# CompVis/stable-diffusion

Hardware: AMD Instinct MI355X
Metric: 512x512 images/sec, SD-v1-4 50-step PLMS CFG=7.5 (higher is better)
Workload: dtype f16

## Files before the change

### stable-diffusion_amd/csrc/conv3halo.hip

```cpp
#include "igemm_dev.h"

namespace sdmi {
namespace {

template <int BM, int BN, int WARPS_M, int WARPS_N, int NS>
__global__ void __launch_bounds__(WARPS_M* WARPS_N * 64) conv3halo_kernel(const IGemmParams p, const int tiles_m,
                                                                           const int tiles_n, const int chunks_per_split) {
#if defined(__HIP_DEVICE_COMPILE__)
  constexpr int NT = WARPS_M * WARPS_N * 64;
  constexpr int RPP = NT / 8;
  constexpr int PB = BN / RPP;
  constexpr int WTM = BM / WARPS_M, WTN = BN / WARPS_N;
  constexpr int TM = WTM / 32, TN = WTN / 32;
  constexpr int HPMAX = (BM / 64 + 2) * 66;
  constexpr int AHP = (HPMAX + RPP - 1) / RPP;
  constexpr int HALO_BYTES = AHP * RPP * 128;
  constexpr int BSTAGE = BN * 128;
  constexpr int LDS_BYTES = 2 * HALO_BYTES + NS * BSTAGE;
  constexpr int LASTA = 10 - NS;
  constexpr int PA = (AHP + LASTA) / (LASTA + 1);
  constexpr int KS = BK / 16;
  constexpr int G = (TM * TN >= 4) ? 1 : 2;
  constexpr int U = KS / G;
  constexpr int MPU = G * TM * TN;
  static_assert(PB >= 1 && TM >= 1 && TN >= 1 && RPP % 16 == 0 && NS >= 2 && NS <= 9, "tile/wave shape");
  static_assert(LDS_BYTES <= 160 * 1024, "LDS budget");

  __shared__ __attribute__((aligned(16))) unsigned char smem[LDS_BYTES];

  const int nblk = gridDim.x;
  const int bid = blockIdx.x;
  const int q8 = nblk >> 3, r8 = nblk & 7, xcd = bid & 7;
  const int wgid = (xcd < r8 ? xcd * (q8 + 1) : r8 * (q8 + 1) + (xcd - r8) * q8) + (bid >> 3);
  const int tiles_mn = tiles_m * tiles_n;
  const int split = wgid / tiles_mn;
  const int tmn = wgid - split * tiles_mn;
  int tile_m, tile_n;
  if (p.tile_n_fastest) { tile_m = tmn / tiles_n; tile_n = tmn - tile_m * tiles_n; }
  else { tile_n = tmn / tiles_m; tile_m = tmn - tile_n * tiles_m; }
  const int m0 = tile_m * BM, n0 = tile_n * BN;
  const int nch = (p.c0 + p.c1 + p.c2) / BK;
  const int c_begin = split * chunks_per_split;
  const int c_end = min(nch, c_begin + chunks_per_split);
  if (c_begin >= c_end) return;

  const int tid = threadIdx.x;
  SDMI_STAMP(dbg_t0);
  const int lane = tid & 63;
  const int wave = tid >> 6;
  const int cpos = tid & 7, lrow = tid >> 3;
  const int gch = cpos ^ ((lrow >> 1) & 7);
  const int wave_u = __builtin_amdgcn_readfirstlane(wave);
  const int wm = wave / WARPS_N, wn = wave - wm * WARPS_N;
  const int l31 = lane & 31, lg = lane >> 5;
  const int rsw = (l31 >> 1) & 7;

  const int W = p.Wout, H = p.Hout, HW = H * W, W2 = W + 2, ld = p.lda0;
  const int bimg = m0 / HW;
  const int THI = p.halo_thi;
  const int HPI = (THI + 2) * W2;
  const int y0 = p.halo_ipt > 1 ? 0 : (m0 - bimg * HW) >> p.log2w;
  const int HP = p.halo_ipt * HPI;
  constexpr int OOB = (int)0x80000000;

  int hvoff[AHP];
#pragma unroll
  for (int q = 0; q < AHP; ++q) {
    const int hp = q * RPP + lrow;
    const int ip = fast_div(hp, p.magic_hpi), hr = hp - ip * HPI;
    const int hy = fast_div(hr, p.magic_w2), hx = hr - hy * W2;
    const int y = y0 + hy - 1, x = hx - 1;
    const bool valid = hp < HP && y >= 0 && y < H && x >= 0 && x < W;
    hvoff[q] = valid ? ((((bimg + ip) * H + y) * W + x) * ld + gch * 8) * 2 : OOB;
  }
  int b_off[PB];
#pragma unroll
  for (int i = 0; i < PB; ++i) {
    const int n = min(n0 + i * RPP + lrow, p.N - 1);
    b_off[i] = (n * p.K + gch * 8) * 2;
  }
  int hr0[TM];
#pragma unroll
  for (int i = 0; i < TM; ++i) {
// ... 4 lines not shown
  const int b_lds = 2 * HALO_BYTES + (wn * WTN + l31) * 128;

  const char* const srcA0 = (const char*)p.a0; const char* const srcA1 = (const char*)p.a1;
  const char* const srcA2 = (const char*)p.a2;
  const __amdgpu_buffer_rsrc_t rsrc_w = __builtin_amdgcn_make_buffer_rsrc((void*)p.w, 0, OOB, 0x00020000);
  const int pc0 = p.c0, pc01 = p.c0 + p.c1;
  struct ChunkSrc { __amdgpu_buffer_rsrc_t rsrc; int soff; };
  auto chunk_src = [&](int c) {
    const int cin0 = c * BK;
    const char* src; int coff;
    if (cin0 < pc0) { src = srcA0; coff = cin0; }
    else if (cin0 < pc01) { src = srcA1; coff = cin0 - pc0; }
    else { src = srcA2; coff = cin0 - pc01; }
    ChunkSrc r; r.rsrc = __builtin_amdgcn_make_buffer_rsrc((void*)src, 0, OOB, 0x00020000); r.soff = coff * 2;
    return r;
  };
  auto issue_halo = [&](const ChunkSrc& cs, int hbuf, int q) {
    auto dst = (__attribute__((address_space(3))) void*)(smem + hbuf * HALO_BYTES + (q * RPP + wave_u * 8) * 128);
    __builtin_amdgcn_raw_ptr_buffer_load_lds(cs.rsrc, dst, 16, hvoff[q], cs.soff, 0, 0);
  };
  auto issue_b = [&](int kt, int stage, int q) {
    auto dst = (__attribute__((address_space(3))) void*)(smem + 2 * HALO_BYTES + stage * BSTAGE + (q * RPP + wave_u * 8) * 128);
    __builtin_amdgcn_raw_ptr_buffer_load_lds(rsrc_w, dst, 16, b_off[q], kt * (BK * 2), 0, SDMI_W_AUX);
  };

  f32x16 acc[TM][TN];
#pragma unroll
  for (int i = 0; i < TM; ++i)
#pragma unroll
    for (int j = 0; j < TN; ++j)
#pragma unroll
      for (int r = 0; r < 16; ++r) acc[i][j][r] = 0.f;

  auto a_base = [&](int i, int ky, int kx, int hbuf) -> int {
    const int rowt = hr0[i] + ky * W2 + kx;
    return hbuf * HALO_BYTES + ((rowt << 7) | ((lg ^ ((rowt >> 1) & 7)) << 4));
  };
  auto read_frags = [&](const int (&ab)[TM], int bstage, int ks, f16x8 (&a)[TM], f16x8 (&b)[TN]) {
#pragma unroll
    for (int i = 0; i < TM; ++i) a[i] = *(const f16x8*)(smem + (ab[i] ^ (ks << 5)));
    const unsigned char* st = smem + bstage * BSTAGE + b_lds + (((ks * 2 + lg) ^ rsw) << 4);
#pragma unroll
    for (int j = 0; j < TN; ++j) b[j] = *(const f16x8*)(st + j * 32 * 128);
  };
  auto mfma_step = [&](const f16x8 (&a)[TM], const f16x8 (&b)[TN]) {
#pragma unroll
    for (int i = 0; i < TM; ++i)
#pragma unroll
      for (int j = 0; j < TN; ++j) acc[i][j] = __builtin_amdgcn_mfma_f32_32x32x16_f16(a[i], b[j], acc[i][j], 0, 0, 0);
  };

  auto a_lo = [](int t) { return t <= LASTA ? (t * PA < AHP ? t * PA : AHP) : AHP; };
  auto a_hi = [](int t) { return t <= LASTA ? ((t + 1) * PA < AHP ? (t + 1) * PA : AHP) : AHP; };
  auto in_flight_ok = [&](int t) {
    int n = 0;
    for (int d = 0; d < NS - 2; ++d) { const int tt = (t - d + 18) % 9; n += a_hi(tt) - a_lo(tt) + PB; }
    return n;
  };

  const int kt_first = c_begin * 9, kt_last = c_end * 9 - 1;
  {
    const ChunkSrc cs = chunk_src(c_begin);
#pragma unroll
    for (int q = 0; q < AHP; ++q) issue_halo(cs, 0, q);
#pragma unroll
    for (int s2 = 0; s2 < NS - 1; ++s2) {
      const int vt = 9 - (NS - 1) + s2;
#pragma unroll
      for (int e = a_lo(vt); e < a_hi(vt); ++e) issue_halo(cs, 0, 0);
#pragma unroll
      for (int q = 0; q < PB; ++q) issue_b(min(kt_first + s2, kt_last), s2, q);
    }
  }
  wait_vmcnt_n(in_flight_ok(8));
  asm volatile("s_waitcnt lgkmcnt(0)\n\ts_barrier" ::: "memory");
  SDMI_STAMP(dbg_t1);
  f16x8 fa[2][G][TM], fb[2][G][TN];
  int ab[TM];
#pragma unroll
  for (int i = 0; i < TM; ++i) ab[i] = a_base(i, 0, 0, 0);
#pragma unroll
  for (int g = 0; g < G; ++g) read_frags(ab, 0, g, fa[0][g], fb[0][g]);

  int cur = 0, nxt = NS - 1, hb = 0;
  for (int c = c_begin; c < c_end; ++c) {
    const ChunkSrc csn = chunk_src(min(c + 1, c_end - 1));
#pragma unroll
    for (int tap = 0; tap < 9; ++tap) {
      const int kt = c * 9 + tap;
      const int tap1 = tap == 8 ? 0 : tap + 1;
      const int hb1 = tap == 8 ? (hb ^ 1) : hb;
      const int cur1 = (cur + 1 == NS) ? 0 : cur + 1;
      int ab1[TM];
#pragma unroll
      for (int i = 0; i < TM; ++i) ab1[i] = a_base(i, tap1 / 3, tap1 % 3, hb1);
      const int alo = a_lo(tap);
      const int na = a_hi(tap) - alo;
      const int npieces = na + PB;
      const int ppu = (npieces + U - 2) / (U - 1);
      const int bt = min(kt + NS - 1, kt_last);
#pragma unroll
      for (int u = 0; u < U; ++u) {
        if (u + 1 < U) {
#pragma unroll
          for (int g = 0; g < G; ++g) read_frags(ab, cur, (u + 1) * G + g, fa[(u + 1) & 1][g], fb[(u + 1) & 1][g]);
#pragma unroll
          for (int e = u * ppu; e < (u + 1) * ppu && e < npieces; ++e) {
            if (e < na) issue_halo(csn, hb ^ 1, alo + e);
            else issue_b(bt, nxt, e - na);
          }
        } else {
          wait_vmcnt_n(in_flight_ok(tap));
          asm volatile("s_waitcnt lgkmcnt(0)\n\ts_barrier" ::: "memory");
#pragma unroll
          for (int g = 0; g < G; ++g) read_frags(ab1, cur1, g, fa[0][g], fb[0][g]);
        }
#pragma unroll
        for (int g = 0; g < G; ++g) mfma_step(fa[u & 1][g], fb[u & 1][g]);
        __builtin_amdgcn_sched_group_barrier(0x100, G * (TM + TN), 0);
#pragma unroll
        for (int e = 0; e < MPU; ++e) {
          __builtin_amdgcn_sched_group_barrier(0x008, 1, 0);
          if (u + 1 < U && e < ppu && u * ppu + e < npieces) __builtin_amdgcn_sched_group_barrier(0x010, 1, 0);
        }
      }
#pragma unroll
      for (int i = 0; i < TM; ++i) ab[i] = ab1[i];
      cur = cur1;
      nxt = (nxt + 1 == NS) ? 0 : nxt + 1;
      hb = hb1;
    }
  }
  wait_vmcnt<0>();
  SDMI_STAMP(dbg_t2);
  igemm_epilogue<BM, BN, WARPS_M, WARPS_N, LDS_BYTES>(p, acc, m0, n0, split, tile_m, tile_n, smem);
#ifdef SDMI_IGEMM_TIMING
  if (p.dbg_times && tid == 0) {
    long long* d = p.dbg_times + 6 * (size_t)blockIdx.x;
    d[0] = dbg_t0; d[1] = dbg_t1; d[2] = dbg_t2; d[4] = (long long)__builtin_readcyclecounter();
  }
#endif
#endif
}

}

bool halo_supported(const IGemmParams& p, int bm) {
  const int W = p.Wout, HW = p.Hout * p.Wout;
  if (p.c0 % BK || p.c1 % BK || p.c2 % BK) return false;
  if (!(p.ksize == 3 && p.stride == 1 && p.pad == 1 && !p.up && p.Hin == p.Hout && p.Win == p.Wout && W >= 8 && W <= 64 &&
        (W & (W - 1)) == 0 && bm % W == 0))
    return false;
  const int cap = (((bm / 64 + 2) * 66 + bm / 4 - 1) / (bm / 4)) * (bm / 4);
  if (bm <= HW) return HW % bm == 0 && (bm / W + 2) * (W + 2) <= cap;
  return bm % HW == 0 && p.M % bm == 0 && (bm / HW) * (p.Hout + 2) * (W + 2) <= cap;
}

template <int BM, int BN, int WARPS_M, int WARPS_N, int NS>
int launch_halo_cfg(const IGemmParams& p, int splitk, hipStream_t stream) {
  SDMI_CHECK(halo_supported(p, BM), "halo-staged conv tile requested for an unsupported shape");
  const int tiles_m = cdiv(p.M, BM), tiles_n = cdiv(p.N, BN);
  const int nch = (p.c0 + p.c1 + p.c2) / BK;
  const int chunks_per_split = cdiv(nch, splitk);
  const int nsplit = cdiv(nch, chunks_per_split);
  IGemmParams q = p;
  q.splitk = nsplit;
  q.tile_n_fastest = tile_order_n_fastest(p);
  q.splitk_fused = 0;
  slab_layout(q, BM, BN, WARPS_M, WARPS_N, nsplit);
  q.epi_vec = epi_vec_ok(p);
  SDMI_CHECK(splitk_ws_need(p, BM, BN, nsplit) <= p.splitk_ws_floats, "split-K workspace too small");
  SDMI_CHECK((int64_t)p.M < (int64_t)65536 * p.Hout * p.Wout, "fast_div_hw: at most 65535 samples per launch");
  q.magic_hw = div_magic_hw(p.Hout * p.Wout);
  q.magic_w = div_magic(p.Wout);
  q.magic_w2 = div_magic(p.Wout + 2);
  q.log2w = 0;
  while ((1 << q.log2w) < p.Wout) ++q.log2w;
  {
    const int HW = p.Hout * p.Wout;
    q.halo_ipt = BM <= HW ? 1 : BM / HW;
    q.halo_thi = BM <= HW ? BM / p.Wout : p.Hout;
    q.magic_hpi = div_magic((q.halo_thi + 2) * (p.Wout + 2));
    const int tpi = q.halo_thi * p.Wout;
    q.log2_tpi = 0;
    while ((1 << q.log2_tpi) < tpi) ++q.log2_tpi;
    if (q.halo_ipt == 1) q.log2_tpi = 30;
  }
  for (int t = 0; t < p.gn_n; ++t) q.gn_magic[t] = div_magic(p.gn_cpg[t]);
  dim3 grid(tiles_m * tiles_n * nsplit), block(WARPS_M * WARPS_N * 64);
  static const int by_shape = env_int("SDMI_PROF_SHAPES", 0);
  std::string pname = std::string("conv3halo_") + std::to_string(BM) + "x" + std::to_string(BN) + "w" +
                      std::to_string(WARPS_M * WARPS_N) + "s" + std::to_string(NS);
  if (by_shape && prof_enabled())
    pname += "_M" + std::to_string(p.M) + "_N" + std::to_string(p.N) + "_K" + std::to_string(p.K) + "_s" + std::to_string(nsplit);
  const double src_pix = (double)p.B * p.Hin * p.Win;
  ProfScope ps(pname.c_str(), 2.0 * p.M * (double)p.N * p.K,
               src_pix * (p.c0 + p.c1) * 2.0 + (double)p.N * p.K * 2.0 + (double)p.M * p.N * ((p.out_f32 ? 4.0 : 0.0) + (p.out_f16 ? 2.0 : 0.0)) +
                   (p.residual ? (double)p.M * p.N * 4.0 : 0.0),
               stream);
  SDMI_LAUNCH((conv3halo_kernel<BM, BN, WARPS_M, WARPS_N, NS>), grid, block, 0, stream, q, tiles_m, tiles_n, chunks_per_split);
  SDMI_HIP_OK(hipGetLastError());
  ps.end();
  if (nsplit > 1) return launch_splitk_reduce(q, nsplit, stream);
  if (q.ln_out) return launch_layernorm(q.out_f32, q.ln_gamma, q.ln_beta, q.ln_out, q.M, q.N, q.ln_eps, stream);
  return 0;
}

int launch_halo_tile(int tile, const IGemmParams& p, int splitk, hipStream_t stream) {
  switch (tile) {
    case 14: return launch_halo_cfg<256, 64, 4, 2, 5>(p, splitk, stream);
    case 15: return launch_halo_cfg<256, 128, 4, 2, 3>(p, splitk, stream);
    case 16: return launch_halo_cfg<128, 64, 2, 2, 8>(p, splitk, stream);
    case 17: return launch_halo_cfg<128, 128, 2, 2, 5>(p, splitk, stream);
    default: return fail("not a halo-staged conv tile id");
  }
// ... 4 lines not shown
```

### stable-diffusion_amd/csrc/gemm_split16.hip

```cpp
#include "igemm_dev.h"

namespace sdmi {
namespace {

template <int BM, int BN, int WARPS_M, int WARPS_N, int NS, bool HALF>
__global__ void __launch_bounds__(WARPS_M* WARPS_N * 64) gemm_split16_kernel(const IGemmParams p, const int tiles_m, const int tiles_n,
                                                                               const int kt_per_split) {
#if defined(__HIP_DEVICE_COMPILE__)
  constexpr int NT = WARPS_M * WARPS_N * 64;
  constexpr int RPP = NT / 8;
  constexpr int A_PASSES = BM / RPP, B_PASSES = BN / RPP;
  constexpr int WTM = BM / WARPS_M, WTN = BN / WARPS_N;
  constexpr int TM = WTM / 32, TN = WTN / 32;
  constexpr int A_BYTES = BM * 128, B_BYTES = BN * 128;
  constexpr int STAGE_BYTES = 2 * (A_BYTES + B_BYTES);
  constexpr int LPT = 2 * (A_PASSES + B_PASSES);
  constexpr int KS = BK / 16;
  constexpr int PPU = (LPT + KS - 2) / (KS - 1);
  static_assert(A_PASSES >= 1 && B_PASSES >= 1 && TM >= 1 && TN >= 1 && RPP % 16 == 0 && NS >= 2, "tile/wave shape");
  static_assert(NS * STAGE_BYTES <= 160 * 1024, "LDS budget");

  __shared__ __attribute__((aligned(16))) unsigned char smem[NS * STAGE_BYTES];

  const int nblk = gridDim.x, bid = blockIdx.x;
// ... 15 lines not shown
  SDMI_STAMP(dbg_t0);
  const int lane = tid & 63, wave = tid >> 6;
  const int cpos = tid & 7, lrow = tid >> 3;
  const int gch = cpos ^ ((lrow >> 1) & 7);
  const int hi_oob = (HALF && gch >= 4) ? (int)0x80000000 : 0;
  const int kt_half = HALF ? nkt - 1 : -1;
  const int wave_u = __builtin_amdgcn_readfirstlane(wave);

  int a_off[A_PASSES], b_off[B_PASSES];
#pragma unroll
  for (int i = 0; i < A_PASSES; ++i) a_off[i] = (min(m0 + i * RPP + lrow, p.M - 1) * p.lda0 + gch * 8) * 2;
#pragma unroll
  for (int i = 0; i < B_PASSES; ++i) b_off[i] = (min(n0 + i * RPP + lrow, p.N - 1) * p.ldw + gch * 8) * 2;
  constexpr int OOB = (int)0x80000000;
  const __amdgpu_buffer_rsrc_t rsrc_hi = __builtin_amdgcn_make_buffer_rsrc((void*)p.a0, 0, OOB, 0x00020000);
  const __amdgpu_buffer_rsrc_t rsrc_lo = __builtin_amdgcn_make_buffer_rsrc((void*)p.a1, 0, OOB, 0x00020000);
  const __amdgpu_buffer_rsrc_t rsrc_w = __builtin_amdgcn_make_buffer_rsrc((void*)p.w, 0, OOB, 0x00020000);
  const int w_lo_off = 2 * p.K * 2;

  auto issue_piece = [&](int kt, int stage, int q) {
    const int soff = kt * (BK * 2);
    const int half = HALF ? (hi_oob & (kt == kt_half ? (int)0x80000000 : 0)) : 0;
    const bool isA = q < 2 * A_PASSES;
    const int qa = isA ? q : q - 2 * A_PASSES;
    const int npass = isA ? A_PASSES : B_PASSES;
    const int hl = qa >= npass ? 1 : 0, pass = qa - hl * npass;
    const unsigned row0 = (isA ? hl * BM : 2 * BM + hl * BN) + pass * RPP + wave_u * 8;
    auto dst = (__attribute__((address_space(3))) void*)(smem + stage * STAGE_BYTES + row0 * 128);
    if (isA) __builtin_amdgcn_raw_ptr_buffer_load_lds(hl ? rsrc_lo : rsrc_hi, dst, 16, a_off[pass] | half, soff, 0, 0);
    else __builtin_amdgcn_raw_ptr_buffer_load_lds(rsrc_w, dst, 16, b_off[pass] | half, soff + (hl ? w_lo_off : 0), 0, SDMI_W_AUX);
  };

  const int wm = wave / WARPS_N, wn = wave - wm * WARPS_N;
  const int l31 = lane & 31, lg = lane >> 5;
  const int rsw = (l31 >> 1) & 7;
  f32x16 acc[TM][TN];
#pragma unroll
  for (int i = 0; i < TM; ++i)
#pragma unroll
    for (int j = 0; j < TN; ++j)
#pragma unroll
      for (int r = 0; r < 16; ++r) acc[i][j][r] = 0.f;

  struct Frags { f16x8 ah[TM], al[TM], bh[TN], bl[TN]; };
  const int a_lds = (wm * WTM + l31) * 128, b_lds = 2 * A_BYTES + (wn * WTN + l31) * 128;
  auto read_frags = [&](int stage, int ks, Frags& f) {
    const unsigned char* st = smem + stage * STAGE_BYTES + (((ks * 2 + lg) ^ rsw) << 4);
#pragma unroll
    for (int i = 0; i < TM; ++i) {
      f.ah[i] = *(const f16x8*)(st + a_lds + i * 32 * 128);
      f.al[i] = *(const f16x8*)(st + a_lds + A_BYTES + i * 32 * 128);
    }
#pragma unroll
    for (int j = 0; j < TN; ++j) {
      f.bh[j] = *(const f16x8*)(st + b_lds + j * 32 * 128);
      f.bl[j] = *(const f16x8*)(st + b_lds + B_BYTES + j * 32 * 128);
    }
  };
  auto mfma_step = [&](const Frags& f) {
#pragma unroll
    for (int i = 0; i < TM; ++i)
#pragma unroll
      for (int j = 0; j < TN; ++j) {
        acc[i][j] = __builtin_amdgcn_mfma_f32_32x32x16_f16(f.ah[i], f.bh[j], acc[i][j], 0, 0, 0);
        acc[i][j] = __builtin_amdgcn_mfma_f32_32x32x16_f16(f.al[i], f.bh[j], acc[i][j], 0, 0, 0);
        acc[i][j] = __builtin_amdgcn_mfma_f32_32x32x16_f16(f.ah[i], f.bl[j], acc[i][j], 0, 0, 0);
      }
  };

  SDMI_STAMP(dbg_t1);
  int ld_kt = kt_begin;
  auto next_kt = [&]() { const int k = ld_kt; if (ld_kt + 1 < kt_end) ++ld_kt; return k; };
#pragma unroll
  for (int s = 0; s < NS - 1; ++s) {
    const int k = next_kt();
#pragma unroll
    for (int q = 0; q < LPT; ++q) issue_piece(k, s, q);
  }
  wait_vmcnt<LPT*(NS - 2)>();
  asm volatile("s_waitcnt lgkmcnt(0)\n\ts_barrier" ::: "memory");
  Frags fr[2];
  read_frags(0, 0, fr[0]);
  int cur = 0, nxt = NS - 1;
  for (int kt = kt_begin; kt < kt_end; ++kt) {
    const int kload = next_kt();
    const int cur1 = (cur + 1 == NS) ? 0 : cur + 1;
#pragma unroll
    for (int u = 0; u < KS; ++u) {
      if (u + 1 < KS) {
        read_frags(cur, u + 1, fr[(u + 1) & 1]);
#pragma unroll
        for (int q = u * PPU; q < (u + 1) * PPU && q < LPT; ++q) issue_piece(kload, nxt, q);
      } else {
        wait_vmcnt<LPT*(NS - 2)>();
        asm volatile("s_waitcnt lgkmcnt(0)\n\ts_barrier" ::: "memory");
        read_frags(cur1, 0, fr[0]);
      }
      mfma_step(fr[u & 1]);
      __builtin_amdgcn_sched_group_barrier(0x100, 2 * (TM + TN), 0);
#pragma unroll
      for (int e = 0; e < 3 * TM * TN; ++e) {
        __builtin_amdgcn_sched_group_barrier(0x008, 1, 0);
        if (u + 1 < KS && e < PPU && u * PPU + e < LPT) __builtin_amdgcn_sched_group_barrier(0x010, 1, 0);
      }
    }
    cur = cur1;
    nxt = (nxt + 1 == NS) ? 0 : nxt + 1;
  }
  wait_vmcnt<0>();
  SDMI_STAMP(dbg_t2);
  igemm_epilogue<BM, BN, WARPS_M, WARPS_N, NS * STAGE_BYTES>(p, acc, m0, n0, split, tile_m, tile_n, smem);
#ifdef SDMI_IGEMM_TIMING
  if (p.dbg_times && tid == 0) {
    long long* d = p.dbg_times + 6 * (size_t)blockIdx.x;
    d[0] = dbg_t0; d[1] = dbg_t1; d[2] = dbg_t2; d[4] = (long long)__builtin_readcyclecounter();
  }
#endif
#endif
}

template <int BM, int BN, int WARPS_M, int WARPS_N, int NS>
int launch_split16_cfg(const IGemmParams& p, int splitk, hipStream_t stream) {
  const int tiles_m = cdiv(p.M, BM), tiles_n = cdiv(p.N, BN);
  const int nkt = igemm_nkt(p);
  const int kt_per_split = cdiv(nkt, splitk);
  const int nsplit = cdiv(nkt, kt_per_split);
  IGemmParams q = p;
  q.nkt = nkt;
  q.splitk = nsplit;
  q.tile_n_fastest = tile_order_n_fastest(p);
  q.splitk_fused = 0;
  slab_layout(q, BM, BN, WARPS_M, WARPS_N, nsplit);
  q.epi_vec = epi_vec_ok(p);
  SDMI_CHECK(splitk_ws_need(p, BM, BN, nsplit) <= p.splitk_ws_floats, "split-K workspace too small");
  SDMI_CHECK((int64_t)p.M < (int64_t)65536 * p.Hout * p.Wout, "fast_div_hw: at most 65535 samples per launch");
  q.magic_hw = div_magic_hw(p.Hout * p.Wout);
  q.magic_w = div_magic(p.Wout);
  for (int t = 0; t < p.gn_n; ++t) q.gn_magic[t] = div_magic(p.gn_cpg[t]);
  dim3 grid(tiles_m * tiles_n * nsplit), block(WARPS_M * WARPS_N * 64);
  static const int by_shape = env_int("SDMI_PROF_SHAPES", 0);
  std::string pname = std::string("gemm_split16_") + std::to_string(BM) + "x" + std::to_string(BN) + "w" +
                      std::to_string(WARPS_M * WARPS_N) + "s" + std::to_string(NS);
  if (by_shape && prof_enabled())
    pname += "_M" + std::to_string(p.M) + "_N" + std::to_string(p.N) + "_K" + std::to_string(p.K) + "_s" + std::to_string(nsplit);
  ProfScope ps(pname.c_str(), 2.0 * p.M * (double)p.N * p.K,
               (double)p.M * p.K * 2.0 + (double)p.N * p.K * 2.0 + (double)p.M * p.N * ((p.out_f32 ? 4.0 : 0.0) + (p.out_f16 ? 2.0 : 0.0)) +
                   (p.residual ? (double)p.M * p.N * 4.0 : 0.0),
               stream, 6.0 * p.M * (double)p.N * p.K);
  if (igemm_has_half(p)) SDMI_LAUNCH((gemm_split16_kernel<BM, BN, WARPS_M, WARPS_N, NS, true>), grid, block, 0, stream, q, tiles_m, tiles_n, kt_per_split);
  else SDMI_LAUNCH((gemm_split16_kernel<BM, BN, WARPS_M, WARPS_N, NS, false>), grid, block, 0, stream, q, tiles_m, tiles_n, kt_per_split);
  SDMI_HIP_OK(hipGetLastError());
  ps.end();
  if (nsplit > 1) return launch_splitk_reduce(q, nsplit, stream);
  if (q.ln_out) return launch_layernorm(q.out_f32, q.ln_gamma, q.ln_beta, q.ln_out, q.M, q.N, q.ln_eps, stream);
  return 0;
}

}

bool split16_tile_supported(int tile) { return tile == 0 || tile == 1 || tile == 2 || tile == 4 || tile == 5 || tile == 8 || tile == 10; }

int launch_split16_tile(int tile, const IGemmParams& p, int splitk, hipStream_t stream) {
  SDMI_CHECK(p.a0 && p.a1 && p.ksize == 1 && p.mode == EPI_PLAIN && p.c1 == 0 && p.c2 == 0 && p.K == p.c0 && p.K % BKH == 0 &&
                 p.lda0 % 8 == 0 && p.ldw % 8 == 0 && p.ldw >= 3 * p.K,
             "split-fp16 GEMM: hi + lo operands, plain epilogue, K % 32 == 0, packed [N][3K] weights");
  switch (tile) {
    case 0: return launch_split16_cfg<128, 128, 2, 2, 2>(p, splitk, stream);
    case 1: return launch_split16_cfg<128, 64, 2, 2, 2>(p, splitk, stream);
    case 2: return launch_split16_cfg<64, 64, 2, 2, 2>(p, splitk, stream);
    case 4: return launch_split16_cfg<128, 64, 2, 2, 3>(p, splitk, stream);
    case 5: return launch_split16_cfg<64, 64, 2, 2, 3>(p, splitk, stream);
    case 8: return launch_split16_cfg<64, 128, 2, 2, 3>(p, splitk, stream);
    case 10: return launch_split16_cfg<64, 64, 2, 2, 4>(p, splitk, stream);
    default: return fail("split-fp16 GEMM: tile id without an instantiation");
  }
}

}
```

### stable-diffusion_amd/csrc/igemm_dev.h

```cpp
#pragma once
#include "common.h"
#include "prof.h"

namespace sdmi {
typedef unsigned u32x4 __attribute__((ext_vector_type(4)));

int launch_splitk_reduce(const IGemmParams& p, int nsplit, hipStream_t stream);
int launch_generic_tile_g0(int tile, const IGemmParams& p, bool dma, int splitk, hipStream_t stream);
int launch_generic_tile_g1(int tile, const IGemmParams& p, bool dma, int splitk, hipStream_t stream);
int launch_generic_tile_g2(int tile, const IGemmParams& p, bool dma, int splitk, hipStream_t stream);
int launch_generic_tile_h0(int tile, const IGemmParams& p, bool dma, int splitk, hipStream_t stream);
int launch_generic_tile_h1(int tile, const IGemmParams& p, bool dma, int splitk, hipStream_t stream);
int launch_generic_tile_h2(int tile, const IGemmParams& p, bool dma, int splitk, hipStream_t stream);

static int env_int(const char* name, int dflt) {
  const char* v = getenv(name);
  return v ? atoi(v) : dflt;
}

namespace {

constexpr int BK = 64;
constexpr int BKH = 32;
static inline int src_chunks(int c) { return (c + BK - 1) / BK; }
static inline bool igemm_has_half(const IGemmParams& p) { return p.split16 ? (p.K % BK != 0) : (p.c0 % BK || p.c1 % BK || p.c2 % BK); }
static inline int igemm_nkt(const IGemmParams& p) {
  if (p.split16) return src_chunks(p.K);
  return p.ksize * p.ksize * (src_chunks(p.c0) + src_chunks(p.c1) + src_chunks(p.c2));
}

#ifdef SDMI_IGEMM_TIMING
#define SDMI_STAMP(name) const long long name = p.dbg_times ? (long long)__builtin_readcyclecounter() : 0
#else
#define SDMI_STAMP(name)
#endif

__device__ __forceinline__ float gelu_erf(float x) {
  const float z = fabsf(x) * 0.70710678118654752440f;
  const float t = __builtin_amdgcn_rcpf(1.0f + 0.3275911f * z);
  const float poly = t * (0.254829592f + t * (-0.284496736f + t * (1.421413741f + t * (-1.453152027f + t * 1.061405429f))));
  const float erf_abs = 1.0f - poly * __expf(-z * z);
  const float erf_v = __builtin_copysignf(erf_abs, x);
  return 0.5f * x * (1.0f + erf_v);
}

__device__ __forceinline__ void wait_vmcnt_n(int n) {
  switch (n) {
#define SDMI_VMCNT_CASE(k) case k: asm volatile("s_waitcnt vmcnt(" #k ")" ::: "memory"); break
    SDMI_VMCNT_CASE(0); SDMI_VMCNT_CASE(1); SDMI_VMCNT_CASE(2); SDMI_VMCNT_CASE(3); SDMI_VMCNT_CASE(4);
    SDMI_VMCNT_CASE(5); SDMI_VMCNT_CASE(6); SDMI_VMCNT_CASE(7); SDMI_VMCNT_CASE(8); SDMI_VMCNT_CASE(9);
    SDMI_VMCNT_CASE(10); SDMI_VMCNT_CASE(11); SDMI_VMCNT_CASE(12); SDMI_VMCNT_CASE(13); SDMI_VMCNT_CASE(14);
    SDMI_VMCNT_CASE(15); SDMI_VMCNT_CASE(16); SDMI_VMCNT_CASE(17); SDMI_VMCNT_CASE(18); SDMI_VMCNT_CASE(19);
    SDMI_VMCNT_CASE(20); SDMI_VMCNT_CASE(21); SDMI_VMCNT_CASE(22); SDMI_VMCNT_CASE(23); SDMI_VMCNT_CASE(24);
    SDMI_VMCNT_CASE(25); SDMI_VMCNT_CASE(26); SDMI_VMCNT_CASE(27); SDMI_VMCNT_CASE(28); SDMI_VMCNT_CASE(29);
    SDMI_VMCNT_CASE(30); SDMI_VMCNT_CASE(31); SDMI_VMCNT_CASE(32); SDMI_VMCNT_CASE(33); SDMI_VMCNT_CASE(34);
    SDMI_VMCNT_CASE(35); SDMI_VMCNT_CASE(36); SDMI_VMCNT_CASE(37); SDMI_VMCNT_CASE(38); SDMI_VMCNT_CASE(39);
    SDMI_VMCNT_CASE(40); SDMI_VMCNT_CASE(41); SDMI_VMCNT_CASE(42); SDMI_VMCNT_CASE(43); SDMI_VMCNT_CASE(44);
    SDMI_VMCNT_CASE(45); SDMI_VMCNT_CASE(46); SDMI_VMCNT_CASE(47); SDMI_VMCNT_CASE(48);
#undef SDMI_VMCNT_CASE
    default: __builtin_trap();
  }
}
template <int N>
__device__ __forceinline__ void wait_vmcnt() {
  static_assert(N >= 0 && N <= 48, "add the literal");
  wait_vmcnt_n(N);
}

enum : int { KIND_1X1 = 0, KIND_3X3 = 1, KIND_3X3_UP = 2 };

__device__ __forceinline__ int fast_div(int m, unsigned long long magic) {
  return (int)(((unsigned long long)(unsigned)m * magic) >> 40);
}
__device__ __forceinline__ int fast_div_hw(int m, unsigned long long magic) {
  return (int)(((unsigned long long)(unsigned)m * magic) >> 48);
}

#if defined(__HIP_DEVICE_COMPILE__)
template <int WTN> constexpr int SLAB_LPR = WTN / 4;
template <int WTN> constexpr int SLAB_RPI = 64 / (WTN / 4);
template <int WTN> constexpr int SLAB_NPASS = 32 / (64 / (WTN / 4));
template <int NWAVES, int WTN, int LDS_BYTES>
constexpr int SLAB_LSTR = (NWAVES * 32 * (WTN + 4) * 4 <= LDS_BYTES) ? WTN + 4 : WTN;
template <int NWAVES, int WTN, int LDS_BYTES>
__device__ __forceinline__ float* slab_base(unsigned char* smem, int wave) {
  static_assert(WTN == 32 || WTN == 64, "lane mapping of the 16-byte epilogue");
  static_assert(NWAVES * 32 * SLAB_LSTR<NWAVES, WTN, LDS_BYTES> * 4 <= LDS_BYTES, "LDS too small for the epilogue slabs");
  return (float*)smem + wave * (32 * SLAB_LSTR<NWAVES, WTN, LDS_BYTES>);
}
template <int TN, int LSTR>
__device__ __forceinline__ void slab_put(float* wl, const f32x16 (&a)[TN], int l31, int lg) {
#pragma unroll
  for (int j = 0; j < TN; ++j)
#pragma unroll
    for (int r = 0; r < 16; ++r) wl[((r & 3) + 8 * (r >> 2) + 4 * lg) * LSTR + j * 32 + l31] = a[j][r];
  asm volatile("s_waitcnt lgkmcnt(0)" ::: "memory");
}
template <int TN, int LSTR>
__device__ __forceinline__ void slab_get(const float* wl, f32x16 (&a)[TN], int l31, int lg) {
  asm volatile("s_waitcnt lgkmcnt(0)" ::: "memory");
#pragma unroll
  for (int j = 0; j < TN; ++j)
#pragma unroll
    for (int r = 0; r < 16; ++r) a[j][r] = wl[((r & 3) + 8 * (r >> 2) + 4 * lg) * LSTR + j * 32 + l31];
  asm volatile("s_waitcnt lgkmcnt(0)" ::: "memory");
}

constexpr int LNF_MAXP = 40;
__device__ __forceinline__ void lnf_request(const IGemmParams& p, int m, float2 (&pv)[LNF_MAXP]) {
  const float2* src = (const float2*)p.lnf_part + m;
#pragma unroll
  for (int j = 0; j < 20; ++j) pv[j] = src[(size_t)min(j, p.lnf_npart - 1) * p.M];
  if (p.lnf_npart > 20) {
#pragma unroll
    for (int j = 20; j < LNF_MAXP; ++j) pv[j] = src[(size_t)min(j, p.lnf_npart - 1) * p.M];
  } else {
#pragma unroll
    for (int j = 20; j < LNF_MAXP; ++j) pv[j] = float2{0.f, 0.f};
  }
}
__device__ __forceinline__ void lnf_finish(const IGemmParams& p, const float2 (&pv)[LNF_MAXP], float* mean, float* rstd) {
  float s = 0.f, q = 0.f;
#pragma unroll
  for (int j = 0; j < LNF_MAXP; ++j)
    if (j < p.lnf_npart) { s += pv[j].x; q += pv[j].y; }
  const float inv_c = 1.0f / (32.0f * (float)p.lnf_npart);
  const float mu = s * inv_c;
  const float var = fmaxf(q * inv_c - mu * mu, 0.f);
  *mean = mu;
  *rstd = 1.0f / sqrtf(var + p.lnf_eps);
}
__device__ __forceinline__ float sum8_dpp(float v) {
  v += __builtin_bit_cast(float, __builtin_amdgcn_update_dpp(0, __builtin_bit_cast(int, v), 0xB1, 0xF, 0xF, true));
  v += __builtin_bit_cast(float, __builtin_amdgcn_update_dpp(0, __builtin_bit_cast(int, v), 0x4E, 0xF, 0xF, true));
  v += __builtin_bit_cast(float, __builtin_amdgcn_update_dpp(0, __builtin_bit_cast(int, v), 0x141, 0xF, 0xF, true));
  return v;
}

template <int BM, int BN, int WARPS_M, int WARPS_N, int LDS_BYTES>
__device__ __forceinline__ void igemm_epilogue(const IGemmParams& p_arg, f32x16 (&acc)[BM / WARPS_M / 32][BN / WARPS_N / 32],
                                               const int m0, const int n0, const int split, const int tile_m,
                                               const int tile_n, unsigned char* smem, const float lnf_mean = 0.f,
                                               const float lnf_rstd = 1.f) {
#ifdef SDMI_IGEMM_TIMING
  IGemmParams p = p_arg;
  if (p.dbg_abl & 1) p.residual = nullptr;
  if (p.dbg_abl & 4) { p.out_f32 = nullptr; p.out_f16 = nullptr; p.out_lo = nullptr; }
#else
  const IGemmParams& p = p_arg;
// ... 505 lines not shown
```

### stable-diffusion_amd/csrc/igemm_kernel.h

```cpp
#pragma once
#include <string>

#include "igemm_dev.h"

namespace sdmi {
namespace {


template <int BM, int BN, int WARPS_M, int WARPS_N, bool DMA, int NS, int KIND, bool HALF = false>
__global__ void __launch_bounds__(WARPS_M* WARPS_N * 64) igemm_kernel(const IGemmParams p, const int tiles_m,
                                                                       const int tiles_n, const int kt_per_split) {
  static_assert(DMA || NS == 2, "the register-staged path is double buffered");
#if defined(__HIP_DEVICE_COMPILE__)
  constexpr bool UP = KIND == KIND_3X3_UP;
  constexpr bool K3 = KIND != KIND_1X1;
  constexpr int NT = WARPS_M * WARPS_N * 64;
  constexpr int RPP = NT / 8;
  constexpr int A_PASSES = BM / RPP;
  constexpr int B_PASSES = BN / RPP;
  constexpr int WTM = BM / WARPS_M, WTN = BN / WARPS_N;
  constexpr int TM = WTM / 32, TN = WTN / 32;
  constexpr int STAGE_BYTES = (BM + BN) * 128;
  static_assert(A_PASSES >= 1 && B_PASSES >= 1 && TM >= 1 && TN >= 1, "tile/wave shape");
  static_assert(RPP % 16 == 0, "swizzle assumes pass offset keeps row bits 1..3");
// ... 136 lines not shown
    else v = a_off[i];
    if constexpr (K3) v = (a_mask[i] & c.tapbit) ? v : OOB;
    else if constexpr (HALF) v |= hi_oob & c.half;
    return v;
  };
  auto b_voff = [&](const TileCursor& c, int i) -> int { return HALF ? (b_off[i] | (hi_oob & c.half)) : b_off[i]; };
  auto issue_piece = [&](const TileCursor& c, int q) {
    const unsigned row0 = (q < A_PASSES ? q * RPP : BM + (q - A_PASSES) * RPP) + wave_u * 8;
    auto dst = (__attribute__((address_space(3))) void*)(smem + c.lds + row0 * 128);
    if (q < A_PASSES) __builtin_amdgcn_raw_ptr_buffer_load_lds(c.rsrc_a, dst, 16, a_voff(c, q), c.a_soff, 0, 0);
    else __builtin_amdgcn_raw_ptr_buffer_load_lds(rsrc_w, dst, 16, b_voff(c, q - A_PASSES), c.b_soff, 0, SDMI_W_AUX);
  };
  auto issue_loads = [&](int stage) {
    const TileCursor c = next_tile(stage);
#pragma unroll
    for (int q = 0; q < A_PASSES + B_PASSES; ++q) {
      if constexpr (DMA) {
        issue_piece(c, q);
      } else {
        typedef int i32x4 __attribute__((ext_vector_type(4)));
        i32x4 v;
        if (q < A_PASSES) v = __builtin_amdgcn_raw_buffer_load_b128(c.rsrc_a, a_voff(c, q), c.a_soff, 0);
        else v = __builtin_amdgcn_raw_buffer_load_b128(rsrc_w, b_voff(c, q - A_PASSES), c.b_soff, 0);
        if (q < A_PASSES) regA[q] = __builtin_bit_cast(f16x8, v);
        else regB[q - A_PASSES] = __builtin_bit_cast(f16x8, v);
      }
    }
  };
  auto commit_regs = [&](int stage) {
    if constexpr (!DMA) {
      unsigned char* As = smem + stage * STAGE_BYTES;
      unsigned char* Bs = As + BM * 128;
#pragma unroll
      for (int i = 0; i < A_PASSES; ++i) *(f16x8*)(As + (i * RPP + lrow) * 128 + cpos * 16) = regA[i];
#pragma unroll
      for (int i = 0; i < B_PASSES; ++i) *(f16x8*)(Bs + (i * RPP + lrow) * 128 + cpos * 16) = regB[i];
    }
  };

  const int wm = wave / WARPS_N, wn = wave - wm * WARPS_N;
  const int l31 = lane & 31, lg = lane >> 5;
  const int rsw = (l31 >> 1) & 7;
  f32x16 acc[TM][TN];
#pragma unroll
  for (int i = 0; i < TM; ++i)
#pragma unroll
    for (int j = 0; j < TN; ++j)
#pragma unroll
      for (int r = 0; r < 16; ++r) acc[i][j][r] = 0.f;

  const int a_lds = (wm * WTM + l31) * 128, b_lds = BM * 128 + (wn * WTN + l31) * 128;
  auto read_frags = [&](int stage, int ks, f16x8 (&a)[TM], f16x8 (&b)[TN]) {
    const unsigned char* st = smem + stage * STAGE_BYTES + (((ks * 2 + lg) ^ rsw) << 4);
#pragma unroll
    for (int i = 0; i < TM; ++i) a[i] = *(const f16x8*)(st + a_lds + i * 32 * 128);
#pragma unroll
    for (int j = 0; j < TN; ++j) b[j] = *(const f16x8*)(st + b_lds + j * 32 * 128);
  };
  auto mfma_step = [&](const f16x8 (&a)[TM], const f16x8 (&b)[TN]) {
#pragma unroll
    for (int i = 0; i < TM; ++i)
#pragma unroll
      for (int j = 0; j < TN; ++j) acc[i][j] = __builtin_amdgcn_mfma_f32_32x32x16_f16(a[i], b[j], acc[i][j], 0, 0, 0);
  };

  SDMI_STAMP(dbg_t1);
  if constexpr (!DMA) { if (lnf_mine) lnf_finish(p, lnf_pv, &lnf_mean, &lnf_rstd); }
  if constexpr (DMA) {
    constexpr int LPT = A_PASSES + B_PASSES;
    constexpr int KS = BK / 16;
    constexpr int G = (TM * TN >= 4) ? 1 : 2;
    constexpr int U = KS / G;
    constexpr int PPU = (LPT + U - 2) / (U - 1);
    constexpr int MPU = G * TM * TN;
#pragma unroll
    for (int s = 0; s < NS - 1; ++s) issue_loads(s);
    if (p.lnf_part) { wait_vmcnt<0>(); if (lnf_mine) lnf_finish(p, lnf_pv, &lnf_mean, &lnf_rstd); }
    wait_vmcnt<LPT*(NS - 2)>();
    asm volatile("s_waitcnt lgkmcnt(0)\n\ts_barrier" ::: "memory");
    f16x8 fa[2][G][TM], fb[2][G][TN];
#pragma unroll
    for (int g = 0; g < G; ++g) read_frags(0, g, fa[0][g], fb[0][g]);
    int cur = 0, nxt = NS - 1;
    for (int kt = kt_begin; kt < kt_end; ++kt) {
      const TileCursor c = next_tile(nxt);
      const int cur1 = (cur + 1 == NS) ? 0 : cur + 1;
#pragma unroll
      for (int u = 0; u < U; ++u) {
        if (u + 1 < U) {
#pragma unroll
          for (int g = 0; g < G; ++g) read_frags(cur, (u + 1) * G + g, fa[(u + 1) & 1][g], fb[(u + 1) & 1][g]);
#pragma unroll
          for (int q = u * PPU; q < (u + 1) * PPU && q < LPT; ++q) issue_piece(c, q);
        } else {
          wait_vmcnt<LPT*(NS - 2)>();
          asm volatile("s_waitcnt lgkmcnt(0)\n\ts_barrier" ::: "memory");
#pragma unroll
          for (int g = 0; g < G; ++g) read_frags(cur1, g, fa[0][g], fb[0][g]);
        }
#pragma unroll
        for (int g = 0; g < G; ++g) mfma_step(fa[u & 1][g], fb[u & 1][g]);
        __builtin_amdgcn_sched_group_barrier(0x100, G * (TM + TN), 0);
#pragma unroll
        for (int e = 0; e < MPU; ++e) {
          __builtin_amdgcn_sched_group_barrier(0x008, 1, 0);
          if (u + 1 < U && e < PPU && u * PPU + e < LPT) __builtin_amdgcn_sched_group_barrier(0x010, 1, 0);
        }
      }
      cur = cur1;
      nxt = (nxt + 1 == NS) ? 0 : nxt + 1;
    }
    wait_vmcnt<0>();
  } else {
    issue_loads(0);
    commit_regs(0);
    for (int kt = kt_begin; kt < kt_end; ++kt) {
      const int cur = (kt - kt_begin) & 1;
      __syncthreads();
      const bool more = (kt + 1 < kt_end);
      if (more) issue_loads(cur ^ 1);
#pragma unroll
      for (int ks = 0; ks < BK / 16; ++ks) {
        f16x8 a[TM], b[TN];
        read_frags(cur, ks, a, b);
        mfma_step(a, b);
      }
      if (more) commit_regs(cur ^ 1);
    }
  }

  SDMI_STAMP(dbg_t2);
  igemm_epilogue<BM, BN, WARPS_M, WARPS_N, NS * STAGE_BYTES>(p, acc, m0, n0, split, tile_m, tile_n, smem, lnf_mean, lnf_rstd);
#ifdef SDMI_IGEMM_TIMING
  if (p.dbg_times && tid == 0) {
    long long* d = p.dbg_times + 6 * (size_t)blockIdx.x;
    d[0] = dbg_t0; d[1] = dbg_t1; d[2] = dbg_t2; d[4] = (long long)__builtin_readcyclecounter();
  }
#endif
#endif
}

template <int BM, int BN, int WARPS_M, int WARPS_N, int NS, bool HALF = false>
int launch_cfg(const IGemmParams& p, bool dma, int splitk, hipStream_t stream) {
  SDMI_CHECK(HALF || (p.c0 % BK == 0 && p.c1 % BK == 0 && p.c2 % BK == 0), "internal: a half k-tile launch on the whole-chunk kernel");
  const int tiles_m = cdiv(p.M, BM), tiles_n = cdiv(p.N, BN);
  const int nkt = igemm_nkt(p);
  const int kt_per_split = cdiv(nkt, splitk);
  const int nsplit = cdiv(nkt, kt_per_split);
  IGemmParams q = p;
  q.nkt = nkt;
  q.splitk = nsplit;
  q.tile_n_fastest = tile_order_n_fastest(p);
  q.splitk_fused = 0;
  slab_layout(q, BM, BN, WARPS_M, WARPS_N, nsplit);
  q.epi_vec = epi_vec_ok(p);
  SDMI_CHECK(splitk_ws_need(p, BM, BN, nsplit) <= p.splitk_ws_floats, "split-K workspace too small");
  SDMI_CHECK((int64_t)p.M < (int64_t)65536 * p.Hout * p.Wout, "fast_div_hw: at most 65535 samples per launch");
  q.magic_hw = div_magic_hw(p.Hout * p.Wout);
  q.magic_w = div_magic(p.Wout);
  for (int t = 0; t < p.gn_n; ++t) q.gn_magic[t] = div_magic(p.gn_cpg[t]);
  dim3 grid(tiles_m * tiles_n * nsplit), block(WARPS_M * WARPS_N * 64);
  static const int by_shape = env_int("SDMI_PROF_SHAPES", 0);
  std::string pname = std::string("igemm_") + std::to_string(BM) + "x" + std::to_string(BN) + "w" +
                      std::to_string(WARPS_M * WARPS_N) + "s" + std::to_string(NS) + (HALF ? "h" : "");
  if (by_shape && prof_enabled())
    pname += "_M" + std::to_string(p.M) + "_N" + std::to_string(p.N) + "_K" + std::to_string(p.K) + "_k" +
             std::to_string(p.ksize) + "_m" + std::to_string(p.mode) + "_s" + std::to_string(nsplit);
  const double src_pix = (double)p.B * p.Hin * p.Win;
  const double out_b = (p.out_f32 ? 4.0 : 0.0) + ((p.out_f16 || p.mode != EPI_PLAIN) ? 2.0 : 0.0);
  const double n_out = p.mode == EPI_GEGLU ? p.N / 2.0 : (double)p.N;
  const int k_alg = p.k_alg > 0 ? p.k_alg : p.K;
  const double cin_alg = p.k_alg > 0 ? (double)p.k_alg : (double)(p.c0 + p.c1 + p.c2);
  ProfScope ps(pname.c_str(), 2.0 * p.M * (double)p.N * k_alg,
               src_pix * cin_alg * 2.0 + (double)p.N * k_alg * 2.0 + (double)p.M * n_out * out_b +
                   (p.residual ? (double)p.M * p.N * 4.0 : 0.0),
               stream, 2.0 * p.M * (double)p.N * p.K);
  const int kind = p.ksize == 1 ? KIND_1X1 : (p.up ? KIND_3X3_UP : KIND_3X3);
#define SDMI_LAUNCH_KIND(K_)                                                                                        \
  do {                                                                                                              \
    if (dma) SDMI_LAUNCH((igemm_kernel<BM, BN, WARPS_M, WARPS_N, true, NS, K_, HALF>), grid, block, 0, stream, q,   \
                                tiles_m, tiles_n, kt_per_split);                                                    \
    else SDMI_LAUNCH((igemm_kernel<BM, BN, WARPS_M, WARPS_N, false, 2, K_, HALF>), grid, block, 0, stream, q,       \
                            tiles_m, tiles_n, kt_per_split);                                                        \
  } while (0)
  if (kind == KIND_1X1) SDMI_LAUNCH_KIND(KIND_1X1);
  else if (kind == KIND_3X3) SDMI_LAUNCH_KIND(KIND_3X3);
  else SDMI_LAUNCH_KIND(KIND_3X3_UP);
#undef SDMI_LAUNCH_KIND
  SDMI_HIP_OK(hipGetLastError());
  ps.end();
  if (nsplit > 1) return launch_splitk_reduce(q, nsplit, stream);
  if (q.ln_out) return launch_layernorm(q.out_f32, q.ln_gamma, q.ln_beta, q.ln_out, q.M, q.N, q.ln_eps, stream);
  return 0;
}
// ... 4 lines not shown
```

Measured before the change: 3.766.

## Drain the multistage load ring without redundant prefetches in the final k-tiles

Splits the main k-loop of the igemm, split16 GEMM and 3x3 halo conv kernels into a steady-state phase and a drain phase. The last NS-1 tiles no longer issue clamped duplicate loads of the final tile, and they use a shrinking vmcnt wait. The halo kernel skips the next-chunk halo prefetch in its last chunk. This removes wasted global-to-LDS traffic and issue slots at the tail of each tile, at the cost of more code paths (a runtime-indexed wait recursion) and larger unrolled code.

```diff
diff --git a/stable-diffusion_amd/csrc/conv3halo.hip b/stable-diffusion_amd/csrc/conv3halo.hip
--- a/stable-diffusion_amd/csrc/conv3halo.hip
+++ b/stable-diffusion_amd/csrc/conv3halo.hip
@@ -1,4 +1,8 @@
 #include "igemm_dev.h"
+
+#ifndef SDMI_RING_DRAIN_HALO
+#define SDMI_RING_DRAIN_HALO SDMI_RING_DRAIN
+#endif
 
 namespace sdmi {
 namespace {
@@ -169,9 +173,17 @@
 #pragma unroll
   for (int g = 0; g < G; ++g) read_frags(ab, 0, g, fa[0][g], fb[0][g]);
 
+  auto in_flight_last = [&](int t) {
+    int n = 0;
+    for (int d = 0; d < NS - 2; ++d) n += (t - d <= 9 - NS) ? PB : 0;
+    return n;
+  };
+
   int cur = 0, nxt = NS - 1, hb = 0;
-  for (int c = c_begin; c < c_end; ++c) {
-    const ChunkSrc csn = chunk_src(min(c + 1, c_end - 1));
+  auto chunk_taps = [&](auto last, const int c) {
+    constexpr bool LAST = decltype(last)::value;
+    ChunkSrc csn;
+    if constexpr (!LAST) csn = chunk_src(SDMI_RING_DRAIN_HALO ? c + 1 : min(c + 1, c_end - 1));
 #pragma unroll
     for (int tap = 0; tap < 9; ++tap) {
       const int kt = c * 9 + tap;
@@ -182,10 +194,10 @@
 #pragma unroll
       for (int i = 0; i < TM; ++i) ab1[i] = a_base(i, tap1 / 3, tap1 % 3, hb1);
       const int alo = a_lo(tap);
-      const int na = a_hi(tap) - alo;
-      const int npieces = na + PB;
+      const int na = LAST ? 0 : a_hi(tap) - alo;
+      const int npieces = na + ((LAST && tap > 9 - NS) ? 0 : PB);
       const int ppu = (npieces + U - 2) / (U - 1);
-      const int bt = min(kt + NS - 1, kt_last);
+      const int bt = SDMI_RING_DRAIN_HALO ? kt + NS - 1 : min(kt + NS - 1, kt_last);
 #pragma unroll
       for (int u = 0; u < U; ++u) {
         if (u + 1 < U) {
@@ -193,11 +205,14 @@
           for (int g = 0; g < G; ++g) read_frags(ab, cur, (u + 1) * G + g, fa[(u + 1) & 1][g], fb[(u + 1) & 1][g]);
 #pragma unroll
           for (int e = u * ppu; e < (u + 1) * ppu && e < npieces; ++e) {
-            if (e < na) issue_halo(csn, hb ^ 1, alo + e);
-            else issue_b(bt, nxt, e - na);
+            if (e < na) {
+              if constexpr (!LAST) issue_halo(csn, hb ^ 1, alo + e);
+            } else {
+              issue_b(bt, nxt, e - na);
+            }
           }
         } else {
-          wait_vmcnt_n(in_flight_ok(tap));
+          wait_vmcnt_n(LAST ? in_flight_last(tap) : in_flight_ok(tap));
           asm volatile("s_waitcnt lgkmcnt(0)\n\ts_barrier" ::: "memory");
 #pragma unroll
           for (int g = 0; g < G; ++g) read_frags(ab1, cur1, g, fa[0][g], fb[0][g]);
@@ -217,7 +232,13 @@
       nxt = (nxt + 1 == NS) ? 0 : nxt + 1;
       hb = hb1;
     }
-  }
+  };
+#if SDMI_RING_DRAIN_HALO
+  for (int c = c_begin; c < c_end - 1; ++c) chunk_taps(std::false_type{}, c);
+  chunk_taps(std::true_type{}, c_end - 1);
+#else
+  for (int c = c_begin; c < c_end; ++c) chunk_taps(std::false_type{}, c);
+#endif
   wait_vmcnt<0>();
   SDMI_STAMP(dbg_t2);
   igemm_epilogue<BM, BN, WARPS_M, WARPS_N, LDS_BYTES>(p, acc, m0, n0, split, tile_m, tile_n, smem);
diff --git a/stable-diffusion_amd/csrc/gemm_split16.hip b/stable-diffusion_amd/csrc/gemm_split16.hip
--- a/stable-diffusion_amd/csrc/gemm_split16.hip
+++ b/stable-diffusion_amd/csrc/gemm_split16.hip
@@ -121,17 +121,21 @@
   Frags fr[2];
   read_frags(0, 0, fr[0]);
   int cur = 0, nxt = NS - 1;
-  for (int kt = kt_begin; kt < kt_end; ++kt) {
-    const int kload = next_kt();
+  auto ktile = [&](auto issue, auto wait) {
+    constexpr bool ISSUE = decltype(issue)::value;
+    int kload = 0;
+    if constexpr (ISSUE) kload = next_kt();
     const int cur1 = (cur + 1 == NS) ? 0 : cur + 1;
 #pragma unroll
     for (int u = 0; u < KS; ++u) {
       if (u + 1 < KS) {
         read_frags(cur, u + 1, fr[(u + 1) & 1]);
-#pragma unroll
-        for (int q = u * PPU; q < (u + 1) * PPU && q < LPT; ++q) issue_piece(kload, nxt, q);
+        if constexpr (ISSUE) {
+#pragma unroll
+          for (int q = u * PPU; q < (u + 1) * PPU && q < LPT; ++q) issue_piece(kload, nxt, q);
+        }
       } else {
-        wait_vmcnt<LPT*(NS - 2)>();
+        wait();
         asm volatile("s_waitcnt lgkmcnt(0)\n\ts_barrier" ::: "memory");
         read_frags(cur1, 0, fr[0]);
       }
@@ -140,12 +144,20 @@
 #pragma unroll
       for (int e = 0; e < 3 * TM * TN; ++e) {
         __builtin_amdgcn_sched_group_barrier(0x008, 1, 0);
-        if (u + 1 < KS && e < PPU && u * PPU + e < LPT) __builtin_amdgcn_sched_group_barrier(0x010, 1, 0);
+        if (ISSUE && u + 1 < KS && e < PPU && u * PPU + e < LPT) __builtin_amdgcn_sched_group_barrier(0x010, 1, 0);
       }
     }
     cur = cur1;
     nxt = (nxt + 1 == NS) ? 0 : nxt + 1;
-  }
+  };
+  auto wait_steady = [] { wait_vmcnt<LPT*(NS - 2)>(); };
+#if SDMI_RING_DRAIN
+  const int nk = kt_end - kt_begin;
+  for (int i = NS - 1; i < nk; ++i) ktile(std::true_type{}, wait_steady);
+  for (int r = min(nk, NS - 1) - 1; r >= 0; --r) ktile(std::false_type{}, [r] { wait_ring_tail<LPT, NS - 2>(r); });
+#else
+  for (int kt = kt_begin; kt < kt_end; ++kt) ktile(std::true_type{}, wait_steady);
+#endif
   wait_vmcnt<0>();
   SDMI_STAMP(dbg_t2);
   igemm_epilogue<BM, BN, WARPS_M, WARPS_N, NS * STAGE_BYTES>(p, acc, m0, n0, split, tile_m, tile_n, smem);
diff --git a/stable-diffusion_amd/csrc/igemm_dev.h b/stable-diffusion_amd/csrc/igemm_dev.h
--- a/stable-diffusion_amd/csrc/igemm_dev.h
+++ b/stable-diffusion_amd/csrc/igemm_dev.h
@@ -1,4 +1,6 @@
 #pragma once
+#include <type_traits>
+
 #include "common.h"
 #include "prof.h"
 
@@ -65,6 +67,19 @@
 __device__ __forceinline__ void wait_vmcnt() {
   static_assert(N >= 0 && N <= 48, "add the literal");
   wait_vmcnt_n(N);
+}
+
+#ifndef SDMI_RING_DRAIN
+#define SDMI_RING_DRAIN 1
+#endif
+template <int LPT, int R>
+__device__ __forceinline__ void wait_ring_tail(int r) {
+  if constexpr (R <= 1) {
+    wait_vmcnt<0>();
+  } else {
+    if (r >= R) wait_vmcnt<LPT*(R - 1)>();
+    else wait_ring_tail<LPT, R - 1>(r);
+  }
 }
 
 enum : int { KIND_1X1 = 0, KIND_3X3 = 1, KIND_3X3_UP = 2 };
diff --git a/stable-diffusion_amd/csrc/igemm_kernel.h b/stable-diffusion_amd/csrc/igemm_kernel.h
--- a/stable-diffusion_amd/csrc/igemm_kernel.h
+++ b/stable-diffusion_amd/csrc/igemm_kernel.h
@@ -242,18 +242,22 @@
 #pragma unroll
     for (int g = 0; g < G; ++g) read_frags(0, g, fa[0][g], fb[0][g]);
     int cur = 0, nxt = NS - 1;
-    for (int kt = kt_begin; kt < kt_end; ++kt) {
-      const TileCursor c = next_tile(nxt);
+    auto ktile = [&](auto issue, auto wait) {
+      constexpr bool ISSUE = decltype(issue)::value;
+      TileCursor c;
+      if constexpr (ISSUE) c = next_tile(nxt);
       const int cur1 = (cur + 1 == NS) ? 0 : cur + 1;
 #pragma unroll
       for (int u = 0; u < U; ++u) {
         if (u + 1 < U) {
 #pragma unroll
           for (int g = 0; g < G; ++g) read_frags(cur, (u + 1) * G + g, fa[(u + 1) & 1][g], fb[(u + 1) & 1][g]);
-#pragma unroll
-          for (int q = u * PPU; q < (u + 1) * PPU && q < LPT; ++q) issue_piece(c, q);
+          if constexpr (ISSUE) {
+#pragma unroll
+            for (int q = u * PPU; q < (u + 1) * PPU && q < LPT; ++q) issue_piece(c, q);
+          }
         } else {
-          wait_vmcnt<LPT*(NS - 2)>();
+          wait();
           asm volatile("s_waitcnt lgkmcnt(0)\n\ts_barrier" ::: "memory");
 #pragma unroll
           for (int g = 0; g < G; ++g) read_frags(cur1, g, fa[0][g], fb[0][g]);
@@ -264,12 +268,20 @@
 #pragma unroll
         for (int e = 0; e < MPU; ++e) {
           __builtin_amdgcn_sched_group_barrier(0x008, 1, 0);
-          if (u + 1 < U && e < PPU && u * PPU + e < LPT) __builtin_amdgcn_sched_group_barrier(0x010, 1, 0);
+          if (ISSUE && u + 1 < U && e < PPU && u * PPU + e < LPT) __builtin_amdgcn_sched_group_barrier(0x010, 1, 0);
         }
       }
       cur = cur1;
       nxt = (nxt + 1 == NS) ? 0 : nxt + 1;
-    }
+    };
+    auto wait_steady = [] { wait_vmcnt<LPT*(NS - 2)>(); };
+#if SDMI_RING_DRAIN
+    const int nk = kt_end - kt_begin;
+    for (int i = NS - 1; i < nk; ++i) ktile(std::true_type{}, wait_steady);
+    for (int r = min(nk, NS - 1) - 1; r >= 0; --r) ktile(std::false_type{}, [r] { wait_ring_tail<LPT, NS - 2>(r); });
+#else
+    for (int kt = kt_begin; kt < kt_end; ++kt) ktile(std::true_type{}, wait_steady);
+#endif
     wait_vmcnt<0>();
   } else {
     issue_loads(0);
```

Result: no change. 3.764 (-0.0%).
